# rlabbe/filterpy

Hardware: AMD Instinct MI355X
Metric: track-steps/sec (predict+update) at dim_x=4 dim_z=2 (higher is better)
Workload: dtype f64

## Files before the change

### filterpy_amd/csrc/rts_mlg.hip

```cpp
#include <stdlib.h>

#include "fk_device.hpp"
#include "fk_math_sym.hpp"
#include "fk_kernel_args.hpp"
#include "fk_ml.hpp"
#include "fk_chunks.hpp"
#include "../../include/filterhip.h"

#ifndef FK_NX
#error "compile with -DFK_NX=<dim_x>"
#endif

#ifndef FK_RMLG8_WAVES
#define FK_RMLG8_WAVES 3
#endif
#define FK_RMLG_CAT_(a, b) a##b
#define FK_RMLG_CAT(a, b) FK_RMLG_CAT_(a, b)

namespace fk {
namespace FK_RMLG_CAT(rmlg_, FK_NX) {

#define FK_OWNER_VAL(v_, k) (((k) / R == 0) ? quad_bcast<0>(v_) : ((k) / R == 1) ? quad_bcast<1>(v_) \
                             : ((k) / R == 2) ? quad_bcast<2>(v_) : quad_bcast<3>(v_))
#define FK_OWNER_ROW(dst, M, k, LEN)                          \
    FK_UNROLL for (int j_ = 0; j_ < (LEN); ++j_) {            \
        const double v_ = M[(k) % R][j_];                     \
        dst[j_] = FK_OWNER_VAL(v_, k);                        \
    }

template <int R, int NX>
__device__ __forceinline__ void store_rows_aos(const double (&M)[R][NX], const unsigned (&row)[R], double *dst, double *tile,
                                               unsigned lane, unsigned valid)
{
    constexpr int EP = NX * NX, UP = 16 * EP / 2;
    using u32x4 = __attribute__((ext_vector_type(4))) unsigned;
    const unsigned q = lane >> 2;
    ml_wave_fence();
    FK_UNROLL for (int r = 0; r < R; ++r)
        FK_UNROLL for (int c = 0; c < NX; ++c) tile[q * EP + row[r] * NX + c] = M[r][c];
    ml_wave_fence();
    const rsrc_t rP = __builtin_amdgcn_make_buffer_rsrc(dst, 0, (int)(valid * (unsigned)EP * 8u), 0x00020000);
    ml_copy_units<UP, 4>(lane, [&](unsigned unit) { return tile + 2u * unit; },
                         [&](unsigned unit, bool ok, const u32x4 &v) {
                             __builtin_amdgcn_raw_buffer_store_b128(v, rP, ok ? unit * 16u : ML_OFF_DROP, 0, 0);
                         });
}

template <int NX, int LAYOUT>
__global__ void __launch_bounds__(BLOCK, (NX <= 8 ? FK_RMLG8_WAVES : NX <= 9 ? 2 : 1))
rts_mlg_kernel(const RtsArgs a)
{
    constexpr int R = (NX + 3) / 4;
    constexpr bool AOS = LAYOUT == LAYOUT_AOS;
    constexpr bool SOA_SLAB = !AOS && NX <= FK_SOA_SLAB_MAX;
    constexpr int REGION = (16 * NX * NX > R * NX * 64) ? 16 * NX * NX : R * NX * 64;
    __shared__ double smem[2 * NX * NX + (BLOCK / 64) * (REGION + 16 * NX)];
    double *tile = smem + 2 * NX * NX + (threadIdx.x >> 6) * REGION;
    double *xpark = smem + 2 * NX * NX + (BLOCK / 64) * REGION + (threadIdx.x >> 2) * NX;
    lds_fill<NX, NX>(smem, a.F, NX, NX, 1.0, threadIdx.x);
    lds_fill<NX, NX>(smem + NX * NX, a.Q, NX, NX, 0.0, threadIdx.x);
    __syncthreads();
    const double *sF = smem, *sQ = smem + NX * NX;

    const long N = a.N, T = a.T;
    const unsigned L = threadIdx.x & 3u;
    const long i0 = a.cnt ? a.i0 : 0, iend = a.cnt ? a.i0 + a.cnt : N;
    long trk = i0 + (long)blockIdx.x * (BLOCK / 4) + (threadIdx.x >> 2);
    if (trk >= iend) trk = iend - 1;
    unsigned estride = AOS ? 8u : (unsigned)N * 8u;
    asm volatile("" : "+s"(estride));
    const unsigned t8 = (unsigned)trk * (AOS ? (unsigned)NX * 8u : 8u);
    const unsigned trk32 = (unsigned)trk;
#define FK_ROWS_HERE()                                                                                     \
    unsigned row[R], off_row[R];                                                                           \
    {                                                                                                      \
        unsigned Lx_ = L, tx_ = trk32;                                                                     \
        asm volatile("" : "+v"(Lx_), "+v"(tx_));                                                           \
        FK_UNROLL for (int r_ = 0; r_ < R; ++r_) {                                                         \
            const unsigned g_ = Lx_ * (unsigned)R + (unsigned)r_;                                          \
            row[r_] = g_ < (unsigned)NX ? g_ : (unsigned)NX - 1u;                                          \
            off_row[r_] = (AOS ? tx_ * (unsigned)(NX * NX) * 8u : tx_ * 8u) + row[r_] * (unsigned)NX * estride; \
        }                                                                                                  \
    }
    const unsigned lane = threadIdx.x & 63u;
    const long w0 = i0 + (long)blockIdx.x * (BLOCK / 4) + (long)wave_index() * 16;
    const unsigned valid = (unsigned)(iend - w0 >= 16 ? 16 : (iend - w0 > 0 ? iend - w0 : 0));
    const long xs_blk = N * NX, ps_blk = N * (long)NX * NX;
    double *park = tile + lane;

#define FK_LOAD_ROWS(base, M)                                                          \
    FK_UNROLL for (int r_ = 0; r_ < R; ++r_) {                                         \
        const MlView v_((base), off_row[r_], estride);                                 \
        FK_UNROLL for (int c_ = 0; c_ < NX; ++c_) M[r_][c_] = v_.load(c_);             \
    }
#define FK_STORE_ROWS(base, step, M)                                                   \
    if constexpr (AOS) {                                                               \
        store_rows_aos<R, NX>(M, row, (base) + ((step) * N + w0) * NX * NX, tile, lane, valid); \
    } else if constexpr (SOA_SLAB) {                                                   \
        ml_store_rows_soa_slab<R, NX, 16>(M, row, (base) + (step) * ps_blk, N, w0, tile, lane, lane >> 2, valid); \
    } else {                                                                           \
        FK_UNROLL for (int r_ = 0; r_ < R; ++r_) {                                     \
            const MlView v_((base) + (step) * ps_blk, off_row[r_], estride);           \
            FK_UNROLL for (int c_ = 0; c_ < NX; ++c_) v_.store(c_, M[r_][c_]);         \
        }                                                                              \
    }
#define FK_PARK(M)                                                                     \
    ml_wave_fence();                                                                   \
    FK_UNROLL for (int r_ = 0; r_ < R; ++r_)                                           \
        FK_UNROLL for (int c_ = 0; c_ < NX; ++c_) park[(r_ * NX + c_) * 64] = M[r_][c_]; \
    ml_wave_fence();

    if (a.cont) {
        FK_ROWS_HERE();
        double xn[NX], Pn[R][NX];
        const MlView vx(a.xs + (T - 1) * xs_blk, t8, estride);
        FK_UNROLL for (int k = 0; k < NX; ++k) xn[k] = vx.load(k);
        FK_LOAD_ROWS(a.Ps_out + (T - 1) * ps_blk, Pn);
        FK_PARK(Pn);
        FK_UNROLL for (int k = 0; k < NX; ++k) xpark[k] = xn[k];
    } else {
        FK_ROWS_HERE();
        double xn[NX], Pn[R][NX];
        const MlView vx(a.Xs + (T - 1) * xs_blk, t8, estride);
        FK_UNROLL for (int k = 0; k < NX; ++k) xn[k] = vx.load(k);
        FK_LOAD_ROWS(a.Ps + (T - 1) * ps_blk, Pn);
        const MlView ox(a.xs + (T - 1) * xs_blk, t8, estride);
        FK_UNROLL for (int k = 0; k < NX; ++k) ox.store(k, xn[k]);
        FK_STORE_ROWS(a.Ps_out, T - 1, Pn);
        FK_STORE_ROWS(a.Pp, T - 1, Pn);
        {
            double Z[R][NX];
            FK_UNROLL for (int r = 0; r < R; ++r)
                FK_UNROLL for (int c = 0; c < NX; ++c) Z[r][c] = 0.0;
            FK_STORE_ROWS(a.K, T - 1, Z);
        }
        FK_PARK(Pn);
        FK_UNROLL for (int k = 0; k < NX; ++k) xpark[k] = xn[k];
    }
    int st = 0;
#define FK_ISYNC()

    _Pragma("nounroll") for (long k = T - 2; k >= 0; --k) {
        double Tm[R][NX];
        FK_ISYNC();
        {
            FK_ROWS_HERE();
            double P[R][NX];
            FK_LOAD_ROWS(a.Ps + k * ps_blk, P);
            double Fr[2][NX];
            FK_UNROLL for (int q = 0; q < NX; ++q) Fr[0][q] = sF[q];
            FK_UNROLL for (int i = 0; i < NX; ++i) {
                if (i + 1 < NX) {
                    FK_UNROLL for (int q = 0; q < NX; ++q) Fr[(i + 1) & 1][q] = sF[(i + 1) * NX + q];
                }
                FK_UNROLL for (int r = 0; r < R; ++r) {
                    double acc = P[r][0] * Fr[i & 1][0];
                    FK_UNROLL for (int q = 1; q < NX; ++q) acc = fma(P[r][q], Fr[i & 1][q], acc);
                    Tm[r][i] = acc;
                }
                FK_STAGE();
            }
        }
        FK_ISYNC();
        {
            FK_ROWS_HERE();
            double Pp[R][NX];
            double fq[2][R];
            FK_UNROLL for (int r = 0; r < R; ++r) fq[0][r] = sF[row[r] * NX];
            FK_UNROLL for (int q = 0; q < NX; ++q) {
                if (q + 1 < NX) {
                    FK_UNROLL for (int r = 0; r < R; ++r) fq[(q + 1) & 1][r] = sF[row[r] * NX + q + 1];
                }
                double Tq[NX];
                FK_OWNER_ROW(Tq, Tm, q, NX);
                FK_UNROLL for (int r = 0; r < R; ++r) {
                    const double f = fq[q & 1][r];
                    FK_UNROLL for (int j = 0; j < NX; ++j) Pp[r][j] = (q == 0) ? f * Tq[j] : fma(f, Tq[j], Pp[r][j]);
                }
                FK_STAGE();
            }
            FK_UNROLL for (int r = 0; r < R; ++r) {
                double Qr[NX];
                FK_UNROLL for (int j = 0; j < NX; ++j) Qr[j] = sQ[row[r] * NX + j];
                FK_STAGE();
                FK_UNROLL for (int j = 0; j < NX; ++j) Pp[r][j] += Qr[j];
            }
            if constexpr (AOS || SOA_SLAB) {
                double Pn[R][NX];
                FK_UNROLL for (int r = 0; r < R; ++r)
                    FK_UNROLL for (int j = 0; j < NX; ++j) Pn[r][j] = park[(r * NX + j) * 64];
                FK_STORE_ROWS(a.Pp, k, Pp);
                ml_wave_fence();
                FK_UNROLL for (int r = 0; r < R; ++r)
                    FK_UNROLL for (int j = 0; j < NX; ++j) park[(r * NX + j) * 64] = Pn[r][j] - Pp[r][j];
                ml_wave_fence();
            } else {
                FK_STORE_ROWS(a.Pp, k, Pp);
                FK_UNROLL for (int r = 0; r < R; ++r)
                    FK_UNROLL for (int j = 0; j < NX; ++j) park[(r * NX + j) * 64] -= Pp[r][j];
            }
            FK_STAGE();
            double d[NX], dinv[NX];
            bool pd = true;
            FK_ISYNC();
            FK_UNROLL for (int j = 0; j < NX; ++j) {
                double Lj[NX];
                FK_UNROLL for (int q = 0; q < NX; ++q)
                    if (q < j) { const double v = Pp[j % R][q]; Lj[q] = FK_OWNER_VAL(v, j); }
                const double ajj = Pp[j % R][j];
                double dj = FK_OWNER_VAL(ajj, j);
                FK_UNROLL for (int q = 0; q < NX; ++q)
                    if (q < j) dj = fma(-Lj[q] * Lj[q], d[q], dj);
                pd = pd && (dj > 0.0);
                d[j] = dj;
                const double di = 1.0 / dj;
                dinv[j] = di;
                FK_UNROLL for (int r = 0; r < R; ++r) {
                    double t = Pp[r][j];
                    FK_UNROLL for (int q = 0; q < NX; ++q)
                        if (q < j) t = fma(-(Pp[r][q] * d[q]), Lj[q], t);
                    Pp[r][j] = row[r] > (unsigned)j ? t * di : Pp[r][j];
                }
                FK_STAGE();
            }
            if (!pd) st |= ST_NOT_PD;
            FK_ISYNC();
            FK_UNROLL for (int i = 1; i < NX; ++i) {
                double Li[NX];
                FK_UNROLL for (int q = 0; q < NX; ++q)
                    if (q < i) { const double v = Pp[i % R][q]; Li[q] = FK_OWNER_VAL(v, i); }
                FK_UNROLL for (int r = 0; r < R; ++r) {
                    double t = Tm[r][i];
                    FK_UNROLL for (int q = 0; q < NX; ++q)
                        if (q < i) t = fma(-Li[q], Tm[r][q], t);
                    Tm[r][i] = t;
                }
                FK_STAGE();
            }
            FK_UNROLL for (int r = 0; r < R; ++r)
                FK_UNROLL for (int i = 0; i < NX; ++i) Tm[r][i] *= dinv[i];
            FK_UNROLL for (int i = NX - 2; i >= 0; --i) {
                double t[R];
                FK_UNROLL for (int r = 0; r < R; ++r) t[r] = Tm[r][i];
                FK_UNROLL for (int q = 0; q < NX; ++q)
                    if (q > i) {
                        const double v = Pp[q % R][i];
                        const double lqi = FK_OWNER_VAL(v, q);
                        FK_UNROLL for (int r = 0; r < R; ++r) t[r] = fma(-lqi, Tm[r][q], t[r]);
                    }
                FK_UNROLL for (int r = 0; r < R; ++r) Tm[r][i] = t[r];
                FK_STAGE();
            }
        }
        FK_ISYNC();
        double E[R][NX];
        {
            double D[R][NX];
            FK_UNROLL for (int r = 0; r < R; ++r)
                FK_UNROLL for (int j = 0; j < NX; ++j) D[r][j] = park[(r * NX + j) * 64];
            FK_UNROLL for (int q = 0; q < NX; ++q) {
                double Dq[NX];
                FK_OWNER_ROW(Dq, D, q, NX);
                FK_UNROLL for (int r = 0; r < R; ++r) {
                    const double kq = Tm[r][q];
                    FK_UNROLL for (int j = 0; j < NX; ++j) E[r][j] = (q == 0) ? kq * Dq[j] : fma(kq, Dq[j], E[r][j]);
                }
                FK_STAGE();
            }
        }
        {
            FK_ROWS_HERE();
            FK_STORE_ROWS(a.K, k, Tm);
        }
        FK_STAGE();
        FK_ISYNC();
        {
            double x[NX], dx[NX];
            {
                const MlView vx(a.Xs + k * xs_blk, t8, estride);
                FK_UNROLL for (int i = 0; i < NX; ++i) x[i] = vx.load(i);
            }
            ml_wave_fence();
            double Fr[2][NX], xpk[NX];
            FK_UNROLL for (int q = 0; q < NX; ++q) Fr[0][q] = sF[q];
            FK_UNROLL for (int i = 0; i < NX; ++i) xpk[i] = xpark[i];
            FK_UNROLL for (int i = 0; i < NX; ++i) {
                if (i + 1 < NX) {
                    FK_UNROLL for (int q = 0; q < NX; ++q) Fr[(i + 1) & 1][q] = sF[(i + 1) * NX + q];
                }
                double acc = Fr[i & 1][0] * x[0];
                FK_UNROLL for (int q = 1; q < NX; ++q) acc = fma(Fr[i & 1][q], x[q], acc);
                dx[i] = xpk[i] - acc;
                FK_STAGE();
            }
            double xn[NX];
            FK_UNROLL for (int j = 0; j < NX; ++j) {
                double Kj[NX];
                FK_OWNER_ROW(Kj, Tm, j, NX);
                double xa = x[j];
                FK_UNROLL for (int q = 0; q < NX; ++q) xa = fma(Kj[q], dx[q], xa);
                xn[j] = xa;
                FK_UNROLL for (int r = 0; r < R; ++r) {
                    double acc = E[r][0] * Kj[0];
                    FK_UNROLL for (int q = 1; q < NX; ++q) acc = fma(E[r][q], Kj[q], acc);
                    park[(r * NX + j) * 64] = acc;
                }
                FK_STAGE();
            }
            const MlView ox(a.xs + k * xs_blk, t8, estride);
            FK_UNROLL for (int i = 0; i < NX; ++i) ox.store(i, xn[i]);
            FK_UNROLL for (int i = 0; i < NX; ++i) xpark[i] = xn[i];
            FK_STAGE();
            FK_ROWS_HERE();
            double P[R][NX];
            FK_LOAD_ROWS(a.Ps + k * ps_blk, P);
            ml_wave_fence();
            FK_UNROLL for (int r = 0; r < R; ++r)
                FK_UNROLL for (int j = 0; j < NX; ++j) P[r][j] += park[(r * NX + j) * 64];
            FK_STORE_ROWS(a.Ps_out, k, P);
            FK_PARK(P);
        }
    }
    if (a.status) {
        double xn[NX];
        FK_UNROLL for (int i = 0; i < NX; ++i) xn[i] = xpark[i];
        bool fin = all_finite<NX>(xn);
        FK_UNROLL for (int r = 0; r < R; ++r)
            FK_UNROLL for (int c = 0; c < NX; ++c) fin = fin && (fabs(park[(r * NX + c) * 64]) <= 1.79769313486231570815e+308);
        int s = st | (fin ? 0 : ST_NONFINITE);
        s |= __builtin_amdgcn_mov_dpp(s, 0xB1, 0xf, 0xf, true);
        s |= __builtin_amdgcn_mov_dpp(s, 0x4E, 0xf, 0xf, true);
        if (L == 0) a.status[trk] = a.status_or ? (a.status[trk] | s) : s;
    }
#undef FK_ROWS_HERE
#undef FK_ISYNC
#undef FK_LOAD_ROWS
#undef FK_STORE_ROWS
#undef FK_PARK
}

}

int FK_RMLG_CAT(launch_rts_mlg_, FK_NX)(const RtsArgs &a, int layout, bool uniform, hipStream_t s)
{
    using namespace FK_RMLG_CAT(rmlg_, FK_NX);
    if (!uniform || a.model_t || a.n != FK_NX || !a.K || !a.Pp || a.T < 2) return 1;
    auto one = [layout](const RtsArgs &b, hipStream_t sb) -> int {
        const long cnt = b.cnt ? b.cnt : b.N;
        const dim3 grid((unsigned)((cnt + BLOCK / 4 - 1) / (BLOCK / 4))), block(BLOCK);
        if (layout == FK_LAYOUT_AOS) hipLaunchKernelGGL((rts_mlg_kernel<FK_NX, LAYOUT_AOS>), grid, block, 0, sb, b);
        else hipLaunchKernelGGL((rts_mlg_kernel<FK_NX, LAYOUT_SOA>), grid, block, 0, sb, b);
        return check_launch("rts_mlg_kernel");
    };
    return rts_chunked_call(a, FK_NX, FK_NX <= 8 ? 3072 : FK_NX <= 9 ? 2048 : 1024, one, s);
}

}
```

Measured before the change: 18.63 billion.

## Coalesce AoS RTS slab loads via buffer b128 and prefetch next step's P and x

For AoS layout with small state dims, the RTS smoother kernel now loads each wave's P and x slabs with whole-wave 128-bit buffer loads staged through LDS, replacing per-row strided loads. It also issues the loads for the next (earlier) time step's P and x before the current step's store and combine work, so that latency overlaps computation. This costs extra registers for the in-flight vectors, more LDS, and additional wave fences. The workload metric is the predict+update filter, while this change touches only the RTS smoother kernel.

```diff
diff --git a/filterpy_amd/csrc/rts_mlg.hip b/filterpy_amd/csrc/rts_mlg.hip
--- a/filterpy_amd/csrc/rts_mlg.hip
+++ b/filterpy_amd/csrc/rts_mlg.hip
@@ -13,6 +13,9 @@
 
 #ifndef FK_RMLG8_WAVES
 #define FK_RMLG8_WAVES 3
+#endif
+#ifndef FK_RMLG_SLAB_LOAD_MAX
+#define FK_RMLG_SLAB_LOAD_MAX 12
 #endif
 #define FK_RMLG_CAT_(a, b) a##b
 #define FK_RMLG_CAT(a, b) FK_RMLG_CAT_(a, b)
@@ -46,6 +49,23 @@
                          });
 }
 
+using ld_u32x4 = __attribute__((ext_vector_type(4))) unsigned;
+template <int U>
+__device__ __forceinline__ void ml_request_units(ld_u32x4 (&v)[(U + 63) / 64], const double *slab, unsigned bytes, unsigned lane)
+{
+    const rsrc_t rs = __builtin_amdgcn_make_buffer_rsrc(const_cast<double *>(slab), 0, (int)bytes, 0x00020000);
+    FK_UNROLL for (int it = 0; it < (U + 63) / 64; ++it)
+        v[it] = __builtin_amdgcn_raw_buffer_load_b128(rs, ((unsigned)it * 64u + lane) * 16u, 0, 0);
+}
+template <int U, bool WHOLE>
+__device__ __forceinline__ void ml_land_units(const ld_u32x4 (&v)[(U + 63) / 64], double *tile, unsigned lane)
+{
+    FK_UNROLL for (int it = 0; it < (U + 63) / 64; ++it) {
+        const unsigned unit = (unsigned)it * 64u + lane;
+        if (WHOLE || (it + 1) * 64 <= U || unit < (unsigned)U) *reinterpret_cast<ld_u32x4 *>(tile + 2u * unit) = v[it];
+    }
+}
+
 template <int NX, int LAYOUT>
 __global__ void __launch_bounds__(BLOCK, (NX <= 8 ? FK_RMLG8_WAVES : NX <= 9 ? 2 : 1))
 rts_mlg_kernel(const RtsArgs a)
@@ -54,9 +74,13 @@
     constexpr bool AOS = LAYOUT == LAYOUT_AOS;
     constexpr bool SOA_SLAB = !AOS && NX <= FK_SOA_SLAB_MAX;
     constexpr int REGION = (16 * NX * NX > R * NX * 64) ? 16 * NX * NX : R * NX * 64;
-    __shared__ double smem[2 * NX * NX + (BLOCK / 64) * (REGION + 16 * NX)];
+    constexpr bool SLABLD = AOS && NX <= FK_RMLG_SLAB_LOAD_MAX;
+    constexpr int UP = 8 * NX * NX, UX = 8 * NX, ITP = (UP + 63) / 64, ITX = (UX + 63) / 64;
+    static_assert(!SLABLD || ITP * 128 <= REGION, "the region holds every unit a whole-wave landing writes");
+    __shared__ double smem[2 * NX * NX + (BLOCK / 64) * (REGION + (SLABLD ? 32 : 16) * NX)];
     double *tile = smem + 2 * NX * NX + (threadIdx.x >> 6) * REGION;
     double *xpark = smem + 2 * NX * NX + (BLOCK / 64) * REGION + (threadIdx.x >> 2) * NX;
+    double *xfil = smem + 2 * NX * NX + (BLOCK / 64) * (REGION + 16 * NX) + (threadIdx.x >> 6) * 16 * NX;
     lds_fill<NX, NX>(smem, a.F, NX, NX, 1.0, threadIdx.x);
     lds_fill<NX, NX>(smem + NX * NX, a.Q, NX, NX, 0.0, threadIdx.x);
     __syncthreads();
@@ -87,12 +111,27 @@
     const unsigned valid = (unsigned)(iend - w0 >= 16 ? 16 : (iend - w0 > 0 ? iend - w0 : 0));
     const long xs_blk = N * NX, ps_blk = N * (long)NX * NX;
     double *park = tile + lane;
+    if (SLABLD && valid == 0) return;
+    const unsigned qc = (lane >> 2) < valid ? (lane >> 2) : valid - 1u;
 
 #define FK_LOAD_ROWS(base, M)                                                          \
     FK_UNROLL for (int r_ = 0; r_ < R; ++r_) {                                         \
         const MlView v_((base), off_row[r_], estride);                                 \
         FK_UNROLL for (int c_ = 0; c_ < NX; ++c_) M[r_][c_] = v_.load(c_);             \
     }
+#define FK_REQUEST_P(step, u) ml_request_units<UP>(u, a.Ps + ((step) * N + w0) * NX * NX, valid * (unsigned)(NX * NX) * 8u, lane)
+#define FK_REQUEST_X(step, u) ml_request_units<UX>(u, a.Xs + ((step) * N + w0) * NX, valid * (unsigned)NX * 8u, lane)
+#define FK_LAND_ROWS(u, M)                                                             \
+    ml_wave_fence();                                                                   \
+    ml_land_units<UP, true>(u, tile, lane);                                            \
+    ml_wave_fence();                                                                   \
+    FK_UNROLL for (int r_ = 0; r_ < R; ++r_)                                           \
+        FK_UNROLL for (int c_ = 0; c_ < NX; ++c_) M[r_][c_] = tile[qc * (unsigned)(NX * NX) + row[r_] * (unsigned)NX + c_]; \
+    ml_wave_fence();
+#define FK_LAND_X(u)                                                                   \
+    ml_wave_fence();                                                                   \
+    ml_land_units<UX, false>(u, xfil, lane);                                           \
+    ml_wave_fence();
 #define FK_STORE_ROWS(base, step, M)                                                   \
     if constexpr (AOS) {                                                               \
         store_rows_aos<R, NX>(M, row, (base) + ((step) * N + w0) * NX * NX, tile, lane, valid); \
@@ -110,12 +149,22 @@
         FK_UNROLL for (int c_ = 0; c_ < NX; ++c_) park[(r_ * NX + c_) * 64] = M[r_][c_]; \
     ml_wave_fence();
 
+    double Pf[SLABLD ? R : 1][SLABLD ? NX : 1];
+#define FK_FIRST_SLABS()                                                               \
+    if constexpr (SLABLD) {                                                            \
+        ld_u32x4 ua[ITP], ux[ITX];                                                     \
+        FK_REQUEST_P(T - 2, ua);                                                       \
+        FK_REQUEST_X(T - 2, ux);                                                       \
+        FK_LAND_ROWS(ua, Pf);                                                          \
+        FK_LAND_X(ux);                                                                 \
+    }
     if (a.cont) {
         FK_ROWS_HERE();
         double xn[NX], Pn[R][NX];
         const MlView vx(a.xs + (T - 1) * xs_blk, t8, estride);
         FK_UNROLL for (int k = 0; k < NX; ++k) xn[k] = vx.load(k);
         FK_LOAD_ROWS(a.Ps_out + (T - 1) * ps_blk, Pn);
+        FK_FIRST_SLABS();
         FK_PARK(Pn);
         FK_UNROLL for (int k = 0; k < NX; ++k) xpark[k] = xn[k];
     } else {
@@ -134,6 +183,7 @@
                 FK_UNROLL for (int c = 0; c < NX; ++c) Z[r][c] = 0.0;
             FK_STORE_ROWS(a.K, T - 1, Z);
         }
+        FK_FIRST_SLABS();
         FK_PARK(Pn);
         FK_UNROLL for (int k = 0; k < NX; ++k) xpark[k] = xn[k];
     }
@@ -146,7 +196,12 @@
         {
             FK_ROWS_HERE();
             double P[R][NX];
-            FK_LOAD_ROWS(a.Ps + k * ps_blk, P);
+            if constexpr (SLABLD) {
+                FK_UNROLL for (int r = 0; r < R; ++r)
+                    FK_UNROLL for (int c = 0; c < NX; ++c) P[r][c] = Pf[r][c];
+            } else {
+                FK_LOAD_ROWS(a.Ps + k * ps_blk, P);
+            }
             double Fr[2][NX];
             FK_UNROLL for (int q = 0; q < NX; ++q) Fr[0][q] = sF[q];
             FK_UNROLL for (int i = 0; i < NX; ++i) {
@@ -276,7 +331,9 @@
         FK_ISYNC();
         {
             double x[NX], dx[NX];
-            {
+            if constexpr (SLABLD) {
+                FK_UNROLL for (int i = 0; i < NX; ++i) x[i] = xfil[qc * (unsigned)NX + i];
+            } else {
                 const MlView vx(a.Xs + k * xs_blk, t8, estride);
                 FK_UNROLL for (int i = 0; i < NX; ++i) x[i] = vx.load(i);
             }
@@ -307,18 +364,43 @@
                 }
                 FK_STAGE();
             }
-            const MlView ox(a.xs + k * xs_blk, t8, estride);
-            FK_UNROLL for (int i = 0; i < NX; ++i) ox.store(i, xn[i]);
-            FK_UNROLL for (int i = 0; i < NX; ++i) xpark[i] = xn[i];
-            FK_STAGE();
-            FK_ROWS_HERE();
-            double P[R][NX];
-            FK_LOAD_ROWS(a.Ps + k * ps_blk, P);
-            ml_wave_fence();
-            FK_UNROLL for (int r = 0; r < R; ++r)
-                FK_UNROLL for (int j = 0; j < NX; ++j) P[r][j] += park[(r * NX + j) * 64];
-            FK_STORE_ROWS(a.Ps_out, k, P);
-            FK_PARK(P);
+            if constexpr (SLABLD) {
+                long kn = k > 0 ? k - 1 : 0;
+                asm volatile("" : "+s"(kn));
+                ld_u32x4 uc[ITP], ua[ITP], ux[ITX];
+                FK_REQUEST_P(k, uc);
+                FK_REQUEST_P(kn, ua);
+                FK_REQUEST_X(kn, ux);
+                const MlView ox(a.xs + k * xs_blk, t8, estride);
+                FK_UNROLL for (int i = 0; i < NX; ++i) ox.store(i, xn[i]);
+                FK_UNROLL for (int i = 0; i < NX; ++i) xpark[i] = xn[i];
+                FK_STAGE();
+                FK_ROWS_HERE();
+                double G[R][NX], P[R][NX];
+                ml_wave_fence();
+                FK_UNROLL for (int r = 0; r < R; ++r)
+                    FK_UNROLL for (int j = 0; j < NX; ++j) G[r][j] = park[(r * NX + j) * 64];
+                FK_LAND_ROWS(uc, P);
+                FK_UNROLL for (int r = 0; r < R; ++r)
+                    FK_UNROLL for (int j = 0; j < NX; ++j) P[r][j] += G[r][j];
+                FK_STORE_ROWS(a.Ps_out, k, P);
+                FK_LAND_ROWS(ua, Pf);
+                FK_LAND_X(ux);
+                FK_PARK(P);
+            } else {
+                const MlView ox(a.xs + k * xs_blk, t8, estride);
+                FK_UNROLL for (int i = 0; i < NX; ++i) ox.store(i, xn[i]);
+                FK_UNROLL for (int i = 0; i < NX; ++i) xpark[i] = xn[i];
+                FK_STAGE();
+                FK_ROWS_HERE();
+                double P[R][NX];
+                FK_LOAD_ROWS(a.Ps + k * ps_blk, P);
+                ml_wave_fence();
+                FK_UNROLL for (int r = 0; r < R; ++r)
+                    FK_UNROLL for (int j = 0; j < NX; ++j) P[r][j] += park[(r * NX + j) * 64];
+                FK_STORE_ROWS(a.Ps_out, k, P);
+                FK_PARK(P);
+            }
         }
     }
     if (a.status) {
@@ -337,6 +419,11 @@
 #undef FK_LOAD_ROWS
 #undef FK_STORE_ROWS
 #undef FK_PARK
+#undef FK_REQUEST_P
+#undef FK_REQUEST_X
+#undef FK_LAND_ROWS
+#undef FK_LAND_X
+#undef FK_FIRST_SLABS
 }
 
 }
```

Result: slower. 18.30 billion (-1.8%).
